# Baverne/VAE-CYCLEGAN-Implementation

Hardware: AMD Instinct MI355X
Metric: train images/sec (256x256 VAE-CycleGAN step) (higher is better)
Workload: dtype f32; 1 GPU; cyclevaegan unpaired, 3x256x256 synthetic summer<->winter, per-GPU batch 8, latent 64 (BASELINE.json configs[3]/[4]); per_gpu_batch=8, global_batch=8, image_size=256, latent_dim=64, parallelism=dp1, init=random (reference init statistics)

## Files before the change

vae-cyclegan-implementation_amd/csrc/conv_igemm.hip:

```cpp
#include "vcg_common.h"
#ifdef VCG_STAMP
#include <stdlib.h>
#endif

struct ConvP {
  const float* a;
  const float* b;
  const float* bias;
  float* out;
  int N, H, W, Cin, Cout, KH, KW, stride, pad, reflect, ups, act;
  int Hl, Wl, Ho, Wo, M, K;
  int cin4, cout4, cout_log;
  FastDiv fd_howo, fd_wo, fd_cin4, fd_cout4, fd_kw, fd_cin;
  int Hc, Wc, Mc, NB;
  FastDiv fd_hcwc, fd_wc;
  int ktiles_total, sk_len, sk_units, sk_ntn, sk_bm_shift, sk_bn_shift;
  int sk_ntr_pb;
  FastDiv fd_sklen;
  int ksplit, kt_per;
  float* slab;
  int adjoint;
  int src_pitch;
  uint32_t a_bytes, b_bytes;
  int dbl_mirror;
// ... 1287 lines not shown
    }
#pragma unroll
    for (int e = 0; e < BE; ++e) {
      vb[e] = bload4(rb, boff[e]);
      if (boff[e] != VCG_OOB) boff[e] += bstep;
    }
  };
  auto store_tiles = [&](int img) {
#pragma unroll
    for (int a = 0; a < AP; ++a) {
      uint2 h, l;
      if (p.a_planes) {
        h = make_uint2(__float_as_uint(va[a].x), __float_as_uint(va[a].y));
        l = make_uint2(__float_as_uint(va[a].z), __float_as_uint(va[a].w));
      } else {
        split4h(va[a], sc.inv_a, h, l);
      }
      const uint32_t o = tr_off<BM>(ps + PS * a, rq * 4);
      *reinterpret_cast<uint2*>(&Xs[img][0][o]) = h;
      *reinterpret_cast<uint2*>(&Xs[img][1][o]) = l;
    }
#pragma unroll
    for (int e = 0; e < BE; ++e) {
      const int idx = tid + NT * e;
      const int pp = idx / (BN / 4), j4 = idx % (BN / 4);
      uint2 h, l;
      split4h(vb[e], sc.inv_b, h, l);
      const uint32_t o = tr_off<BN>(pp, j4 * 4);
      *reinterpret_cast<uint2*>(&Ds[img][0][o]) = h;
      *reinterpret_cast<uint2*>(&Ds[img][1][o]) = l;
    }
  };
  const int tq = (lane & 15) >> 2, tp = lane & 3, tcol = 16 * ((lane >> 4) & 1) + 4 * tp;

  if (kt_begin < kt_end) {
    load_tiles(kt_begin);
    store_tiles(0);
  }
  __syncthreads();
  VCG_STAMP_AT(1);
  for (int kt = kt_begin; kt < kt_end; ++kt) {
    const int img = (kt - kt_begin) & 1;
    if (kt + 1 < kt_end) load_tiles(kt + 1);
#pragma unroll
    for (int s2 = 0; s2 < 2; ++s2) {
      const int row0 = 16 * s2 + 8 * lh + tq;
      f16x8 af[VCG_NP][MI], bfr[VCG_NP][NI];
#pragma unroll
      for (int pc = 0; pc < VCG_NP; ++pc) {
#pragma unroll
        for (int i = 0; i < MI; ++i) af[pc][i] = tr_frag<BM>(Xs[img][pc], row0, wm * (BM / WR) + i * 32 + tcol);
#pragma unroll
        for (int j = 0; j < NI; ++j) bfr[pc][j] = tr_frag<BN>(Ds[img][pc], row0, wn * (BN / 2) + j * 32 + tcol);
      }
#pragma unroll
      for (int i = 0; i < MI; ++i)
#pragma unroll
        for (int j = 0; j < NI; ++j) {
          f32x16 c = lo[i][j];
          c = VCG_MFMA(af[1][i], bfr[0][j], c);
          c = VCG_MFMA(af[0][i], bfr[1][j], c);
          lo[i][j] = c;
          acc[i][j] = VCG_MFMA(af[0][i], bfr[0][j], acc[i][j]);
        }
    }
    if (kt + 1 < kt_end) store_tiles(img ^ 1);
    __syncthreads();
  }
#pragma unroll
  for (int i = 0; i < MI; ++i)
#pragma unroll
    for (int j = 0; j < NI; ++j) acc[i][j] += lo[i][j];
  VCG_STAMP_AT(2);
  const int part = wg - (int)fd_div((uint32_t)(tile * p.ktiles_total), p.fd_sklen);
  float* slab = p.out + ((size_t)part * p.nbatch + zb) * p.K * p.Cout;
#pragma unroll
  for (int j = 0; j < NI; ++j) {
    const int co = n0 + wn * (BN / 2) + j * 32 + l31;
    if (co >= p.Cout) continue;
#pragma unroll
    for (int i = 0; i < MI; ++i) {
#pragma unroll
      for (int e = 0; e < 16; ++e) {
        const int row = (e & 3) + 8 * (e >> 2) + 4 * lh;
        const int Rr = r0 + wm * (BM / WR) + i * 32 + row;
        if (Rr < p.K) slab[(size_t)Rr * p.Cout + co] = acc[i][j][e] * sc.out;
      }
    }
  }
  unit += kt_end - kt_begin;
  if (unit < unit_end) __syncthreads();
  }
  VCG_STAMP_AT(3);
}

__device__ __forceinline__ int sk_parts(const ConvP& p, int R, int co) {
  const int tile = (R >> p.sk_bm_shift) * p.sk_ntn + (co >> p.sk_bn_shift);
  const uint32_t u0 = (uint32_t)(tile * p.ktiles_total);
  return (int)(fd_div(u0 + (uint32_t)p.ktiles_total - 1u, p.fd_sklen) - fd_div(u0, p.fd_sklen)) + 1;
}

__global__ __launch_bounds__(256) void k_slab_sum(const float* __restrict__ slabs, float* __restrict__ out,
                                                  size_t total4, ConvP p, int per_group) {
  const int g = blockIdx.y;
  const int z0 = g * per_group;
  const int c4 = p.Cout / 4;
  for (size_t i = (size_t)blockIdx.x * blockDim.x + threadIdx.x; i < total4; i += (size_t)gridDim.x * blockDim.x) {
    const int R = (int)(i / c4), co = (int)(i - (size_t)R * c4) * 4;
    int z1 = z0 + per_group;
    const int np = sk_parts(p, R, co);
    if (z1 > np) z1 = np;
    float4 s = f4zero();
    for (int z = z0; z < z1; ++z) f4add(s, reinterpret_cast<const float4*>(slabs)[(size_t)z * total4 + i]);
    reinterpret_cast<float4*>(out)[(size_t)g * total4 + i] = s;
  }
}

__global__ __launch_bounds__(256) void k_wgrad_scatter(const float* __restrict__ slabs, float* __restrict__ gw,
                                                       ConvP p, int nsplit, int cin_log, int cout_log) {
  const size_t total = (size_t)p.K * p.Cout;
  const int U2 = p.ups * p.ups, KK = p.KH * p.KW;
  for (size_t idx = (size_t)blockIdx.x * blockDim.x + threadIdx.x; idx < total;
       idx += (size_t)gridDim.x * blockDim.x) {
    const uint32_t R = (uint32_t)(idx / p.Cout);
    const int co = (int)(idx - (size_t)R * p.Cout);
    const uint32_t t = R / (uint32_t)p.Cin;
    const int c = (int)(R - t * (uint32_t)p.Cin);
    if (co >= cout_log || c >= cin_log) continue;
    const int tap9 = (int)t / U2, ph = (int)t - tap9 * U2;
    const int nz = nsplit ? nsplit : sk_parts(p, (int)R, co);
    float s = 0.f;
    for (int z = 0; z < nz; ++z) s += slabs[(size_t)z * total + idx];
    gw[((size_t)co * (cin_log * U2) + (size_t)c * U2 + ph) * KK + tap9] += s;
  }
}

__global__ __launch_bounds__(256) void k_wgrad_scatter_swapped(const float* __restrict__ slabs, float* __restrict__ gw,
                                                               ConvP p, int T, int C, int nsplit, int cin_real,
                                                               int cout_real) {
  const size_t total = (size_t)T * 4 * C;
  for (size_t idx = (size_t)blockIdx.x * blockDim.x + threadIdx.x; idx < total;
       idx += (size_t)gridDim.x * blockDim.x) {
    const int c = (int)(idx % C);
    const int R = (int)(idx / C);
    const int t = R >> 2, j = R & 3;
    if (j >= cout_real || c >= cin_real) continue;
    const int nz = nsplit ? nsplit : sk_parts(p, R, c);
    float s = 0.f;
    for (int z = 0; z < nz; ++z) s += slabs[(size_t)z * total + idx];
    gw[((size_t)j * cin_real + c) * T + t] += s;
  }
}

__global__ __launch_bounds__(256) void k_wgrad_reduce(const float* __restrict__ slabs, float* __restrict__ gw,
                                                      ConvP p, int nsplit, int cin_log, int cout_log) {
  extern __shared__ __attribute__((aligned(16))) float tile[];
  const int U2 = p.ups * p.ups, KK = p.KH * p.KW, T = KK * U2;
  const int co0 = blockIdx.x * 32, c0 = blockIdx.y * 8;
  const int cl_ = threadIdx.x >> 5, col = threadIdx.x & 31;
  const size_t total = (size_t)p.K * p.Cout;
  {
    const int c = c0 + cl_, co = co0 + col;
    const bool ok = c < p.Cin && co < p.Cout;
    for (int t = 0; t < T; ++t) {
      float s = 0.f;
      if (ok) {
        const size_t idx = ((size_t)t * p.Cin + c) * p.Cout + co;
        const int nz = nsplit ? nsplit : sk_parts(p, t * p.Cin + c, co);
        for (int z = 0; z < nz; ++z) s += slabs[(size_t)z * total + idx];
      }
      tile[(t * 8 + cl_) * 33 + col] = s;
    }
  }
  __syncthreads();
  const int wid = threadIdx.x >> 6, lane = threadIdx.x & 63;
  const int cinL = cin_log * U2;
  const int run = 8 * U2 * KK;
  for (int idx = lane; idx < 8 * run; idx += 64) {
    const int j = idx / run, q = idx - j * run;
    const int colw = wid * 8 + j, co = co0 + colw;
    const int clq = q / KK, tap9 = q - clq * KK;
    const int c_local = clq / U2, ph = clq - c_local * U2;
    const int c = c0 + c_local;
    if (co >= cout_log || c >= cin_log) continue;
    const int t = tap9 * U2 + ph;
    const size_t o = ((size_t)co * cinL + (size_t)c * U2 + ph) * KK + tap9;
    gw[o] += tile[(t * 8 + c_local) * 33 + colw];
  }
}

__global__ __launch_bounds__(256) void k_wino_wgrad_reduce(const float* __restrict__ slabs, float* __restrict__ gw, ConvP p,
                                                           int Cin, int ups, int cin_log, int cout_log) {
  __shared__ float tile[9 * 8 * 65];
  const int U2 = ups * ups, KK = 9;
  const int co0 = blockIdx.x * 64, c0 = blockIdx.y * 8, ph = blockIdx.z;
  const int cl_ = threadIdx.x >> 5, col = (threadIdx.x & 31) * 2;
  const size_t plane = (size_t)p.nbatch * p.K * p.Cout;
  {
    const int c = c0 + cl_, co = co0 + col;
    const bool ok = c < Cin;
    float2 s[16];
    int nz[16], nzmax = 0;
#pragma unroll
    for (int xi = 0; xi < 16; ++xi) {
      nz[xi] = ok ? sk_parts(p, xi * p.K + ph * Cin + c, co) : 0;
      nzmax = nz[xi] > nzmax ? nz[xi] : nzmax;
      s[xi] = make_float2(0.f, 0.f);
    }
    const float* src = slabs + (size_t)(ph * Cin + (ok ? c : 0)) * p.Cout + co;
    const size_t xstride = (size_t)p.K * p.Cout;
    for (int z = 0; z < nzmax; ++z) {
      float2 v[16];
#pragma unroll
      for (int xi = 0; xi < 16; ++xi)
        v[xi] = z < nz[xi] ? *reinterpret_cast<const float2*>(src + (size_t)z * plane + (size_t)xi * xstride) : make_float2(0.f, 0.f);
#pragma unroll
      for (int xi = 0; xi < 16; ++xi) { s[xi].x += v[xi].x; s[xi].y += v[xi].y; }
    }
#pragma unroll
    for (int e = 0; e < 2; ++e) {
      float h[3][4];
#pragma unroll
      for (int b = 0; b < 4; ++b) {
        const float s0 = e ? s[0 + b].y : s[0 + b].x, s1 = e ? s[4 + b].y : s[4 + b].x;
        const float s2 = e ? s[8 + b].y : s[8 + b].x, s3 = e ? s[12 + b].y : s[12 + b].x;
        h[0][b] = s0 + 0.5f * (s1 + s2);
        h[1][b] = 0.5f * (s1 - s2);
        h[2][b] = 0.5f * (s1 + s2) + s3;
      }
#pragma unroll
      for (int a = 0; a < 3; ++a) {
        tile[((a * 3 + 0) * 8 + cl_) * 65 + col + e] = h[a][0] + 0.5f * (h[a][1] + h[a][2]);
        tile[((a * 3 + 1) * 8 + cl_) * 65 + col + e] = 0.5f * (h[a][1] - h[a][2]);
        tile[((a * 3 + 2) * 8 + cl_) * 65 + col + e] = 0.5f * (h[a][1] + h[a][2]) + h[a][3];
      }
    }
  }
  __syncthreads();
  const int wid = threadIdx.x >> 6, lane = threadIdx.x & 63;
  const int cinL = cin_log * U2;
  for (int idx = lane; idx < 16 * 8 * KK; idx += 64) {
    const int j = idx / (8 * KK), q = idx - j * (8 * KK);
    const int colw = wid * 16 + j, co = co0 + colw;
    const int c_local = q / KK, tap9 = q - c_local * KK;
    const int c = c0 + c_local;
    if (co >= cout_log || c >= cin_log) continue;
    gw[((size_t)co * cinL + (size_t)c * U2 + ph) * KK + tap9] += tile[(tap9 * 8 + c_local) * 65 + colw];
  }
}

__device__ __forceinline__ void pack_header(const ConvP& p, uint32_t* hdr) {
  if (blockIdx.x == 0 && blockIdx.y == 0 && threadIdx.x < 64) {
    const uint32_t b = vcg_amax_bits(p.amax_b);
    if (threadIdx.x == 0) *hdr = b;
  }
}
__global__ void k_pack_weight(const float* __restrict__ w, float* __restrict__ wf, ConvP p, int cin_log,
                              int cout_log, uint32_t* hdr) {
  pack_header(p, hdr);
  const size_t total = (size_t)p.K * p.Cout;
  for (size_t idx = (size_t)blockIdx.x * blockDim.x + threadIdx.x; idx < total;
       idx += (size_t)gridDim.x * blockDim.x) {
    uint32_t R = (uint32_t)(idx / p.Cout);
    int co = (int)(idx - (size_t)R * p.Cout);
    uint32_t tap = R / (uint32_t)p.Cin;
    int c = (int)(R - tap * (uint32_t)p.Cin);
    float v = 0.f;
    if (co < cout_log && c < cin_log) {
      int ii = 0, jj = 0;
      if (p.ups == 2) { jj = tap & 1; ii = (tap >> 1) & 1; tap >>= 2; }
      int kh = (int)tap / p.KW, kw = (int)tap % p.KW;
      int cl = (p.ups == 2) ? (c * 4 + ii * 2 + jj) : c;
      int cinL = (p.ups == 2) ? cin_log * 4 : cin_log;
      v = w[(((size_t)co * cinL + cl) * p.KH + kh) * p.KW + kw];
    }
    wf[idx] = v;
  }
}

__global__ __launch_bounds__(256) void k_pack_weight_t(const float* __restrict__ w, float* __restrict__ wf, ConvP p,
                                                       int cin_log, int cout_log, uint32_t* hdr) {
  extern __shared__ __attribute__((aligned(16))) float tile[];
  pack_header(p, hdr);
  const int U2 = p.ups * p.ups, KK = p.KH * p.KW, T = KK * U2;
  const int co0 = blockIdx.x * 32, c0 = blockIdx.y * 8;
  const int wid = threadIdx.x >> 6, lane = threadIdx.x & 63;
  const int cinL = cin_log * U2;
  const int run = 8 * U2 * KK;
  for (int j = 0; j < 8; ++j) {
    const int colw = wid * 8 + j, co = co0 + colw;
    for (int q = lane; q < run; q += 64) {
      const int clq = q / KK, tap9 = q - clq * KK;
      const int c_local = clq / U2, ph = clq - c_local * U2;
      const int c = c0 + c_local;
      const int t = tap9 * U2 + ph;
      float v = 0.f;
      if (co < cout_log && c < cin_log) v = w[((size_t)co * cinL + (size_t)c * U2 + ph) * KK + tap9];
      tile[(t * 8 + c_local) * 33 + colw] = v;
    }
  }
  __syncthreads();
  const int cl_ = threadIdx.x >> 5, col = threadIdx.x & 31;
  const int c = c0 + cl_, co = co0 + col;
  if (c < p.Cin && co < p.Cout)
    for (int t = 0; t < T; ++t) wf[((size_t)t * p.Cin + c) * p.Cout + co] = tile[(t * 8 + cl_) * 33 + col];
}

template <bool DGRAD>
__global__ __launch_bounds__(256) void k_pack_planes(const float* __restrict__ w, unsigned short* __restrict__ bp, ConvP p, int cin_log,
                                                     int cout_log) {
  float psc, pinv;
  vcg_scale_of(vcg_amax_bits(p.amax_b), p.amax_b.shift, psc, pinv);
  const int U2 = p.ups * p.ups, KK = p.KH * p.KW;
  const int cinL = cin_log * U2;
  const int KB = (p.K + 31) / 32, CB = p.Cout / 32;
  const size_t total = DGRAD ? (size_t)KK * U2 * p.Cin * (p.Cout / 4) : (size_t)p.Cout * KB * 8;
  for (size_t idx = (size_t)blockIdx.x * blockDim.x + threadIdx.x; idx < total; idx += (size_t)gridDim.x * blockDim.x) {
    float v[4] = {0.f, 0.f, 0.f, 0.f};
    unsigned short* o;
    if (DGRAD) {
      const size_t row = idx / (p.Cout / 4);
      const int co0 = (int)(idx - row * (p.Cout / 4)) * 4;
      const int NB = U2 * p.Cin;
      const int tapfull = (int)(row / NB), J = (int)(row - (size_t)tapfull * NB);
      const int q = J / p.Cin, c = J - q * p.Cin;
      const int kh = tapfull / p.KW, kw = tapfull - kh * p.KW;
      if (c < cin_log) {
#pragma unroll
        for (int e = 0; e < 4; ++e)
          if (co0 + e < cout_log) v[e] = w[(((size_t)(co0 + e) * cinL + (size_t)c * U2 + q) * p.KH + kh) * p.KW + kw];
      }
      o = bp + (row * CB + co0 / 32) * VCG_PBLK + (co0 & 31);
    } else {
      const int co = (int)(idx / ((size_t)KB * 8));
      const int k0 = (int)(idx - (size_t)co * KB * 8) * 4;
      if (co < cout_log && k0 < p.K) {
        uint32_t tap = (uint32_t)k0 / (uint32_t)p.Cin;
        const int c = k0 - (int)tap * p.Cin;
        int ii = 0, jj = 0;
        if (p.ups == 2) { jj = tap & 1; ii = (tap >> 1) & 1; tap >>= 2; }
        const int kh = (int)tap / p.KW, kw = (int)tap % p.KW;
#pragma unroll
        for (int e = 0; e < 4; ++e)
          if (c + e < cin_log) {
            const int cl = (p.ups == 2) ? ((c + e) * 4 + ii * 2 + jj) : c + e;
            v[e] = w[(((size_t)co * cinL + cl) * p.KH + kh) * p.KW + kw];
          }
      }
      o = bp + ((size_t)co * KB + k0 / 32) * VCG_PBLK + (k0 & 31);
    }
    uint2 h, l;
    split4h(make_float4(v[0], v[1], v[2], v[3]), pinv, h, l);
    *reinterpret_cast<uint2*>(o) = h;
    *reinterpret_cast<uint2*>(o + 32) = l;
  }
}

__global__ __launch_bounds__(256) void k_colsum_partial(const float* __restrict__ dy, float* __restrict__ part,
                                                        int M, int C, int rows_per_chunk, int TC) {
  __shared__ float4 red[256];
  const int TP = 256 / TC;
  const int tc = threadIdx.x % TC, tp = threadIdx.x / TC;
  const int c4 = blockIdx.x * TC + tc;
  const int mb = blockIdx.y * rows_per_chunk;
  int me = mb + rows_per_chunk;
  if (me > M) me = M;
  float4 s = make_float4(0.f, 0.f, 0.f, 0.f), s2 = s, s3 = s, s4 = s;
  if (c4 * 4 < C) {
    const float* base = dy + (size_t)c4 * 4;
    int m = mb + tp;
    for (; m + 3 * TP < me; m += 4 * TP) {
      float4 a = ldg4(base + (size_t)m * C), b = ldg4(base + (size_t)(m + TP) * C);
      float4 c = ldg4(base + (size_t)(m + 2 * TP) * C), d = ldg4(base + (size_t)(m + 3 * TP) * C);
      f4add(s, a); f4add(s2, b); f4add(s3, c); f4add(s4, d);
    }
    for (; m < me; m += TP) f4add(s, ldg4(base + (size_t)m * C));
    f4add(s, s2); f4add(s3, s4); f4add(s, s3);
  }
  red[threadIdx.x] = s;
  __syncthreads();
  if (tp == 0 && c4 * 4 < C) {
    for (int k = 1; k < TP; ++k) f4add(s, red[k * TC + tc]);
    float* o = part + (size_t)blockIdx.y * C + c4 * 4;
    *reinterpret_cast<float2*>(o) = make_float2(s.x, s.y);
    *reinterpret_cast<float2*>(o + 2) = make_float2(s.z, s.w);
  }
}
__global__ __launch_bounds__(256) void k_colsum_final(const float* __restrict__ part, float* __restrict__ out, int C,
                                                      int nchunk, int c_log) {
  __shared__ float red[32][8];
  const int il = threadIdx.x & 7, kl = threadIdx.x >> 3;
  const int c = blockIdx.x * 8 + il;
  float s0 = 0.f, s1 = 0.f, s2 = 0.f, s3 = 0.f;
  if (c < c_log) {
    int k = kl;
    for (; k + 96 < nchunk; k += 128) {
      s0 += part[(size_t)k * C + c];
      s1 += part[(size_t)(k + 32) * C + c];
      s2 += part[(size_t)(k + 64) * C + c];
      s3 += part[(size_t)(k + 96) * C + c];
    }
// ... 426 lines not shown
  VCG_CHECK_ARG(pre_mean && pre_rstd, "vcg_conv_fwd_in_pre: null statistics");
  VCG_CHECK_ARG(pre_act >= VCG_ACT_NONE && pre_act <= VCG_ACT_SIGMOID, "vcg_conv_fwd_in_pre: bad activation %d", pre_act);
  const VcgPre pre = {pre_mean, pre_rstd, pre_act};
  (void)vcg_take_hint_x();
  return conv_fwd_in_impl(t_prev, wf, bias, y, mean, rstd, eps, saved, cd, ws, ws_bytes, stream, &pre);
}

extern "C" int vcg_conv_reads_wf(const int32_t* cd) {
  ConvGeom g;
  if (vcg_conv_geom(cd, &g, "vcg_conv_reads_wf")) return 1;
  return (plan_fwd(g).reads_wf || plan_dgrad(g).reads_wf) ? 1 : 0;
}

extern "C" size_t vcg_conv_dgrad_workspace(const int32_t* cd) {
  ConvGeom g;
  if (vcg_conv_geom(cd, &g, "vcg_conv_dgrad_workspace")) return 0;
  return plan_dgrad(g).ws;
}

static KernelRef dgrad_kernel(const DgradPlan& pl) {
  const int bm = pl.t.bm, bn = pl.t.bn;
  if (pl.path == DGRAD_SPLIT_PLANES && bn == 128) return {k_conv_dgrad_split<128, 2>, "k_conv_dgrad_split<128, 2>"};
  if (pl.path == DGRAD_SPLIT_PLANES) return {k_conv_dgrad_split<64, 2>, "k_conv_dgrad_split<64, 2>"};
  if (pl.path == DGRAD_SPLIT32) return {k_conv_dgrad_split<32, 1>, "k_conv_dgrad_split<32, 1>"};
  if (pl.path == DGRAD_SPLIT64_NOPLANES) return {k_conv_dgrad_split<64, 2, false>, "k_conv_dgrad_split<64, 2>"};
  const char* const name = "k_conv_dgrad<fp32 MFMA>";
  if (bn == 32) return {k_conv_dgrad<128, 32, 1>, name};
  if (bm == 128 && bn == 128) return {k_conv_dgrad<128, 128>, name};
  if (bm == 128 && bn == 64) return {k_conv_dgrad<128, 64>, name};
  if (bm == 64 && bn == 128) return {k_conv_dgrad<64, 128>, name};
  return {k_conv_dgrad<64, 64>, name};
}
static void dgrad_setup(const ConvGeom& g, const DgradPlan& pl, void* ws, ConvP& p) {
  p.Hc = g.Hl / g.stride; p.Wc = g.Wl / g.stride; p.Mc = g.N * p.Hc * p.Wc;
  p.NB = g.ups * g.ups * g.Cin;
  p.fd_hcwc = make_fastdiv((uint32_t)(p.Hc * p.Wc));
  p.fd_wc = make_fastdiv((uint32_t)p.Wc);
  auto dbl = [&](int L) { int lo = 1 > L - 1 - g.pad ? 1 : L - 1 - g.pad, hi = g.pad < L - 2 ? g.pad : L - 2; return lo <= hi; };
  p.dbl_mirror = g.reflect && (dbl(g.Hl) || dbl(g.Wl));
  if (pl.t.nsplit > 1) { p.ksplit = pl.t.nsplit; p.kt_per = pl.t.kt_per; p.slab = (float*)ws; }
}

extern "C" int vcg_conv_dgrad(const float* dy, const float* wf, float* dx, const int32_t* cd, void* ws,
                              size_t ws_bytes, void* stream) {
  (void)vcg_take_hint_x();
  const uint64_t dy_handle = vcg_take_hint_dy();
  ConvGeom g;
  if (vcg_conv_geom(cd, &g, "vcg_conv_dgrad")) return -1;
  VCG_CHECK_ARG(dy && wf && dx, "vcg_conv_dgrad: null pointer");
  const DgradPlan pl = plan_dgrad(g);
  VCG_CHECK_ARG(pl.path != DGRAD_UNSUPPORTED, "vcg_conv_dgrad: input %dx%d not divisible by stride", g.Hl, g.Wl);
  VCG_CHECK_ARG(g.stride == 1 || g.ups == 1, "vcg_conv_dgrad: stride 2 with ups 2 unsupported");
  const PackLayout L = pack_layout(g);
  const void* const w_amax = wf + L.hdr;
  hipStream_t st = (hipStream_t)stream;
  if (pl.path == DGRAD_THIN_FOLD) return vcg_thin_fold_dgrad(g, dy, wf + L.wkd, w_amax, dx, ws, ws_bytes, st, dy_handle);
  if (pl.path == DGRAD_THIN) return vcg_thin_dgrad(g, dy, wf, dx, ws, ws_bytes, st);
  if (pl.path == DGRAD_WINO) return vcg_wino_dgrad(g, dy, wf + L.ud, w_amax, dx, ws, ws_bytes, st, dy_handle);
  if (pl.path == DGRAD_SLAB) return vcg_slab_dgrad(g, dy, wf + L.wfd, (L.hdr - L.wfd) * 4, w_amax, dx, ws, ws_bytes, st, dy_handle);
  ConvP p; fill_params(g, p);
  p.a = dy; p.b = wf; p.out = dx;
  if (set_extents(p, (unsigned long long)g.M * g.Cout * 4, (unsigned long long)g.K * g.Cout * 4,
                  "vcg_conv_dgrad: tensor extents must stay below 2 GiB")) return -1;
  const int nsplit = pl.t.nsplit;
  if (nsplit > 1) VCG_CHECK_ARG(ws && ws_bytes >= pl.ws, "vcg_conv_dgrad: workspace too small (%zu)", ws_bytes);
  dgrad_setup(g, pl, ws, p);
  if (pl.path == DGRAD_SPLIT_PLANES) { p.b = wf + L.wfd; p.b_bytes = (uint32_t)((L.hdr - L.wfd) * 4); }
  if (pl.path != DGRAD_FP32) {
    if (vcg_operand_amax(dy, (size_t)g.M * g.Cout, dy_handle, g.reflect ? 4 : 0, st, &p.amax_a)) return -2;
    p.amax_b = vcg_amax_stored(w_amax);
  }
  {
    const KernelRef k = dgrad_kernel(pl);
    dim3 grid((p.Mc + pl.t.bm - 1) / pl.t.bm, (p.NB + pl.t.bn - 1) / pl.t.bn, nsplit * g.stride * g.stride);
    VcgProfScope prof(k.name, 2.0 * g.M * (double)g.K * g.Cout, st);
    hipLaunchKernelGGL(k.fn, grid, dim3(256), 0, st, p);
  }
  if (nsplit > 1)
    hipLaunchKernelGGL(k_splitk_finish, dim3(ew_grid((size_t)g.N * g.H * g.W * g.Cin / 4)), dim3(256), 0, st,
                       (const float*)ws, (const float*)nullptr, dx, (size_t)g.N * g.H * g.W, g.Cin, nsplit, g.Cin,
                       (int)VCG_ACT_NONE);
  VCG_LAUNCH_CHECK("vcg_conv_dgrad");
  return 0;
}

struct WgradPlan { int bm, bn, grid, len, parts, total, ntr, ntn; };
static WgradPlan wgrad_plan(const ConvGeom& g, int batches = 1) {
  WgradPlan best_p = {};
  const int total = (g.M + BK - 1) / BK;
  struct Cand { int bm, bn, resident; double t_step; };
  const Cand cands[4] = {{256, 128, 1, 4.3}, {128, 128, 2, 5.1}, {128, 64, 3, 4.7}, {64, 64, 5, 4.8}};
  double best = 1e30;
  int force = 0;
#ifdef VCG_STAMP
  { const char* e = getenv("VCG_WGRAD_BM"); force = e ? atoi(e) : 0; }
#endif
  for (int ci = 0; ci < 4; ++ci) {
    const Cand& c = cands[ci];
    if (force ? c.bm != force : c.bm == 256) continue;
    if (c.bn == 128 && g.Cout <= 64) continue;
    if (c.bm >= 128 && g.K <= 64) continue;
    if (c.bm == 256 && g.K < 512) continue;
    if (batches > 1 && g.K % c.bm) continue;
    const int ntr = ((g.K + c.bm - 1) / c.bm) * batches, ntn = (g.Cout + c.bn - 1) / c.bn;
    const long long tiles = (long long)ntr * ntn, units = tiles * total;
    if (units >= (1LL << 30)) continue;
    const long long slots = 256LL * c.resident;
    long long len = (units + slots - 1) / slots;
    if (len < 8) len = units < 8 ? units : 8;
    const long long grid = (units + len - 1) / len;
    const int parts = (int)((total + len - 1) / len) + 1;
    double t = (double)len * c.t_step + (double)(grid + tiles) * c.bm * c.bn * 8.0 / 3.0e6;
    if (t < best * 0.97) {
      best = t;
      best_p = {c.bm, c.bn, (int)grid, (int)len, parts, total, ntr, ntn};
    }
  }
  return best_p;
}

static void stream_k_setup(const WgradPlan& wp, ConvP& p) {
  p.ktiles_total = wp.total; p.sk_len = wp.len; p.sk_units = wp.ntr * wp.ntn * wp.total; p.sk_ntn = wp.ntn;
  p.sk_bm_shift = wp.bm == 256 ? 8 : wp.bm == 128 ? 7 : 6; p.sk_bn_shift = wp.bn == 128 ? 7 : 6;
  p.fd_sklen = make_fastdiv((uint32_t)wp.len);
}
static void launch_stream_k(const WgradPlan& wp, const ConvP& p, double flops, hipStream_t st) {
  const int bm = wp.bm, bn = wp.bn;
  const KernelRef k = bm == 128 && bn == 128  ? KernelRef{k_conv_wgrad_split<128>, "k_conv_wgrad_split<128>"}
                      : bm == 128 && bn == 64 ? KernelRef{k_conv_wgrad_split<64>, "k_conv_wgrad_split<64>"}
                      : bm == 64 && bn == 128 ? KernelRef{k_conv_wgrad<64, 128>, "k_conv_wgrad<fp32 MFMA>"}
                      : bm == 64              ? KernelRef{k_conv_wgrad<64, 64>, "k_conv_wgrad<fp32 MFMA>"}
                                              : KernelRef{k_conv_wgrad<256, 128, 512>, "k_conv_wgrad<fp32 MFMA>"};
  VcgProfScope prof(k.name, flops, st);
  hipLaunchKernelGGL(k.fn, dim3(wp.grid), dim3(bm == 256 ? 512 : 256), 0, st, p);
}

static const int kMaxDirectSlabs = 24;

static void colsum_plan(const ConvGeom& g, int& tc, int& cgroups, int& rows, int& nchunk) {
  int c4 = g.Cout / 4;
  tc = 1;
  while (tc * 2 <= c4 && tc * 2 <= 256) tc *= 2;
  cgroups = (c4 + tc - 1) / tc;
  int tp = 256 / tc;
  long long want = 512 / cgroups;
  if (want < 1) want = 1;
  long long r = (g.M + want - 1) / want;
  if (r < 4LL * tp) r = 4LL * tp;
  rows = (int)r;
  nchunk = (g.M + rows - 1) / rows;
}

static ConvGeom wino_gemm_geom(const ConvGeom& g, int T) { return gemm_geom(T, g.ups * g.ups * g.Cin, g.Cout); }
static int wino_wgrad_reduce(const ConvGeom& g, const ConvP& p, const float* dU, float* gw_oihw, hipStream_t st) {
  hipLaunchKernelGGL(k_wino_wgrad_reduce, dim3(g.Cout / 64, (g.Cin + 7) / 8, g.ups * g.ups), dim3(256), 0, st, dU, gw_oihw, p, g.Cin,
                     g.ups, g.cin_log, g.cout_log);
  VCG_LAUNCH_CHECK("vcg_conv_wgrad(winograd reduce)");
  return 0;
}
static size_t wino_core_bytes(const ConvGeom& q, const WgradPlan& wp) { return (size_t)wp.parts * 16 * q.K * q.Cout * sizeof(float) + 256; }
size_t vcg_wino_wgrad_core_workspace(const ConvGeom& g, int T) {
  const ConvGeom q = wino_gemm_geom(g, T);
  return wino_core_bytes(q, wgrad_plan(q, 16));
}
int vcg_wino_wgrad_core(const ConvGeom& g, const float* V, const float* dM, int T, float* gw_oihw, void* ws, size_t ws_bytes,
                        hipStream_t st, const VcgAmax& amax_v, const VcgAmax& amax_dm) {
  const ConvGeom q = wino_gemm_geom(g, T);
  const WgradPlan wp = wgrad_plan(q, 16);
  VCG_CHECK_ARG(wp.grid > 0, "vcg_conv_wgrad: no launch plan for the Winograd path");
  VCG_CHECK_ARG(ws_bytes >= wino_core_bytes(q, wp), "vcg_conv_wgrad: Winograd slab workspace too small");
  ConvP p; fill_params(q, p);
  p.a = V; p.b = dM; p.out = (float*)ws;
  p.amax_a = amax_v; p.amax_b = amax_dm;
  p.a_planes = 1;
  VCG_CHECK_ARG(wp.bm == 128 && q.K % 32 == 0, "vcg_conv_wgrad: pre-split V needs the split-operand tile");
  p.a_bytes = (uint32_t)((size_t)T * q.K * 4); p.b_bytes = (uint32_t)((size_t)T * q.Cout * 4);
  p.nbatch = 16; p.a_bstride = (uint32_t)((size_t)T * q.K); p.b_bstride = (uint32_t)((size_t)T * q.Cout);
  stream_k_setup(wp, p);
  p.sk_ntr_pb = wp.ntr / 16;
  launch_stream_k(wp, p, 2.0 * 16 * (double)T * q.K * q.Cout, st);
  VCG_LAUNCH_CHECK("vcg_conv_wgrad(winograd gemm)");
  return wino_wgrad_reduce(g, p, (const float*)ws, gw_oihw, st);
}

int vcg_wino_wgrad_reduce_one(const ConvGeom& g, const float* dU, float* gw_oihw, hipStream_t st) {
  const ConvGeom q = wino_gemm_geom(g, 32);
  ConvP p; fill_params(q, p);
  p.nbatch = 16;
  p.ktiles_total = 1; p.sk_len = 1; p.sk_ntn = 1; p.sk_bm_shift = 30; p.sk_bn_shift = 30;
  p.fd_sklen = make_fastdiv(1u);
  return wino_wgrad_reduce(g, p, dU, gw_oihw, st);
}

static bool wgrad_swapped_ok(const ConvGeom& g) {
  return g.Cout == 4 && g.stride == 1 && g.ups == 1 && g.Ho == g.H && g.Wo == g.W && g.Cin >= 32;
}
static ConvGeom swapped_geom(const ConvGeom& g) {
  ConvGeom s = g;
  s.Cin = 4; s.Cout = g.Cin; s.cin_log = g.cout_log; s.cout_log = g.cin_log;
  s.taps = g.KH * g.KW; s.K = s.taps * 4; s.M = g.N * g.H * g.W; s.act = 0;
  return s;
}

enum WgradPath { WGRAD_WINO, WGRAD_RING, WGRAD_SWAPPED, WGRAD_STREAM_K };
enum WgradReduce { WRED_SCATTER, WRED_SCATTER_SWAPPED, WRED_REDUCE };
struct WgradWs { size_t slabs_off, slabs_bytes, groups_off, colsum_off, total; };
struct WgradRoute {
  WgradPath path;
  ConvGeom g;
  WgradPlan wp;
  bool slab_sum;
  WgradReduce reduce;
  WgradWs ws;
};
static WgradRoute plan_wgrad(const ConvGeom& g) {
  WgradRoute r = {};
  r.g = g;
  int tc, cgroups, rows, nchunk;
  colsum_plan(g, tc, cgroups, rows, nchunk);
  const size_t cols = (size_t)nchunk * g.Cout * sizeof(float);
  size_t groups = 0;
  if (vcg_wino_wgrad_ok(g)) { r.path = WGRAD_WINO; r.ws.slabs_bytes = vcg_wino_wgrad_workspace(g); }
  else if (vcg_ring_wgrad_ok(g)) { r.path = WGRAD_RING; r.ws.slabs_bytes = vcg_ring_wgrad_workspace(g); }
  else {
    const bool swapped = wgrad_swapped_ok(g);
    r.path = swapped ? WGRAD_SWAPPED : WGRAD_STREAM_K;
    if (swapped) r.g = swapped_geom(g);
    r.wp = wgrad_plan(r.g);
    const size_t totalw = (size_t)r.g.K * r.g.Cout;
    r.ws.slabs_bytes = (size_t)r.wp.parts * totalw * sizeof(float);
    groups = (size_t)16 * totalw * sizeof(float);
    r.slab_sum = r.wp.parts > kMaxDirectSlabs;
    const size_t lds = (size_t)r.g.taps * 8 * 33 * sizeof(float);
    r.reduce = swapped ? WRED_SCATTER_SWAPPED : (totalw < (1u << 20) || lds > 64 * 1024) ? WRED_SCATTER : WRED_REDUCE;
  }
  r.ws.groups_off = up256(r.ws.slabs_bytes);
  r.ws.colsum_off = r.ws.groups_off + up256(groups);
  r.ws.total = r.ws.colsum_off + cols + 1024;
  if (groups) r.ws.total -= r.ws.groups_off - r.ws.slabs_bytes;
  return r;
}

extern "C" size_t vcg_conv_wgrad_workspace(const int32_t* cd) {
  ConvGeom g;
  if (vcg_conv_geom(cd, &g, "vcg_conv_wgrad_workspace")) return 0;
  return plan_wgrad(g).ws.total;
}

static int launch_colsum(const ConvGeom& gorig, const float* dy, float* gbias, float* part, hipStream_t st) {
  int tc, cgroups, rows, nchunk;
  colsum_plan(gorig, tc, cgroups, rows, nchunk);
  hipLaunchKernelGGL(k_colsum_partial, dim3(cgroups, nchunk), dim3(256), 0, st, dy, part, gorig.M, gorig.Cout, rows, tc);
  hipLaunchKernelGGL(k_colsum_final, dim3((gorig.cout_log + 7) / 8), dim3(256), 0, st, (const float*)part, gbias,
                     gorig.Cout, nchunk, gorig.cout_log);
  VCG_LAUNCH_CHECK("vcg_conv_wgrad(bias)");
  return 0;
}

extern "C" int vcg_conv_wgrad_saved(const float* x, const float* dy, float* gw_oihw, float* gbias, const float* saved,
                                    const int32_t* cd, void* ws, size_t ws_bytes, void* stream) {
  const uint64_t x_handle = vcg_take_hint_x(), dy_handle = vcg_take_hint_dy();
  ConvGeom gorig;
  if (vcg_conv_geom(cd, &gorig, "vcg_conv_wgrad")) return -1;
  VCG_CHECK_ARG(x && dy && gw_oihw && ws, "vcg_conv_wgrad: null pointer");
  const WgradRoute r = plan_wgrad(gorig);
  VCG_CHECK_ARG(ws_bytes >= r.ws.total, "vcg_conv_wgrad: workspace %zu < %zu", ws_bytes, r.ws.total);
  hipStream_t st = (hipStream_t)stream;
  float* const colsum = (float*)((char*)ws + r.ws.colsum_off);
  if (r.path == WGRAD_WINO || r.path == WGRAD_RING) {
    if (r.path == WGRAD_WINO ? vcg_wino_wgrad(gorig, x, dy, gw_oihw, ws, r.ws.slabs_bytes, st, saved, x_handle, dy_handle)
                             : vcg_ring_wgrad(gorig, x, dy, gw_oihw, ws, r.ws.slabs_bytes, st, x_handle, dy_handle))
      return -2;
    return gbias ? launch_colsum(gorig, dy, gbias, colsum, st) : 0;
  }
  const bool swapped = r.path == WGRAD_SWAPPED;
  const ConvGeom& g = r.g;
  const WgradPlan& wp = r.wp;
  ConvP p; fill_params(g, p);
  p.a = x; p.b = dy; p.out = (float*)((char*)ws + r.ws.slabs_off);
  if (swapped) { p.a = dy; p.b = x; p.adjoint = 1; p.src_pitch = 4; }
  if (set_extents(p, swapped ? (unsigned long long)gorig.M * 4 * 4 : (unsigned long long)g.N * g.H * g.W * g.Cin * 4,
                  (unsigned long long)g.M * g.Cout * 4, "vcg_conv_wgrad: tensor extents must stay below 2 GiB")) return -1;
  stream_k_setup(wp, p);
  if (wp.bm == 128) {
    if (vcg_operand_amax(p.a, (size_t)p.a_bytes / 4, swapped ? dy_handle : x_handle, (swapped && gorig.reflect) ? 4 : 0, st, &p.amax_a) ||
        vcg_operand_amax(p.b, (size_t)p.b_bytes / 4, swapped ? x_handle : dy_handle, 0, st, &p.amax_b))
      return -2;
  }
  launch_stream_k(wp, p, 2.0 * g.M * (double)g.K * g.Cout, st);
  VCG_LAUNCH_CHECK("vcg_conv_wgrad");
  const size_t totalw = (size_t)g.K * g.Cout;
  const float* src = p.out;
  int ns = 0;
  if (r.slab_sum) {
    float* grp = (float*)((char*)ws + r.ws.groups_off);
    int per_group = (wp.parts + 15) / 16;
    int G = (wp.parts + per_group - 1) / per_group;
    size_t total4 = totalw / 4;
    int bx = (int)((total4 + 255) / 256); if (bx > 1024) bx = 1024;
    hipLaunchKernelGGL(k_slab_sum, dim3(bx, G), dim3(256), 0, st, src, grp, total4, p, per_group);
    src = grp;
    ns = G;
  }
  int blocks = (int)((totalw + 255) / 256); if (blocks > 4096) blocks = 4096;
  if (r.reduce == WRED_SCATTER_SWAPPED)
    hipLaunchKernelGGL(k_wgrad_scatter_swapped, dim3(blocks), dim3(256), 0, st, src, gw_oihw, p, g.KH * g.KW, g.Cout, ns,
                       gorig.cin_log, gorig.cout_log);
  else if (r.reduce == WRED_SCATTER)
    hipLaunchKernelGGL(k_wgrad_scatter, dim3(blocks), dim3(256), 0, st, src, gw_oihw, p, ns, g.cin_log, g.cout_log);
  else
    hipLaunchKernelGGL(k_wgrad_reduce, dim3((g.Cout + 31) / 32, (g.Cin + 7) / 8), dim3(256), (size_t)g.taps * 8 * 33 * sizeof(float),
                       st, src, gw_oihw, p, ns, g.cin_log, g.cout_log);
  VCG_LAUNCH_CHECK("vcg_conv_wgrad(reduce)");
  return gbias ? launch_colsum(gorig, dy, gbias, colsum, st) : 0;
}
extern "C" int vcg_conv_wgrad(const float* x, const float* dy, float* gw_oihw, float* gbias,
                              const int32_t* cd, void* ws, size_t ws_bytes, void* stream) {
  return vcg_conv_wgrad_saved(x, dy, gw_oihw, gbias, nullptr, cd, ws, ws_bytes, stream);
}
```

Baseline: 256.1 images/s.

## Restage wgrad reduce tiles in output order for vectorized aligned gradient accumulation

Rewrites the weight-gradient reduce kernels so the shared-memory tile is laid out in the destination OIHW order, with per-row alignment phase padding. A shared helper can then accumulate into the gradient with float4 read-modify-writes instead of scattered scalar adds. The generic reduce also batches 8 taps per slab pass. The Winograd reduce now covers all phases in one block with float4 loads and gains a specialized single-part variant that skips the split bookkeeping. This targets uncoalesced global writes and the extra launch dimension, at the cost of more complex index math and a risk of alignment or edge-case bugs.

New measurement: 253.8 images/s. Within noise of the previous version (-0.9%).

```diff
diff --git a/vae-cyclegan-implementation_amd/csrc/conv_igemm.hip b/vae-cyclegan-implementation_amd/csrc/conv_igemm.hip
--- a/vae-cyclegan-implementation_amd/csrc/conv_igemm.hip
+++ b/vae-cyclegan-implementation_amd/csrc/conv_igemm.hip
@@ -1463,101 +1463,150 @@
   }
 }
 
+__device__ __forceinline__ int wgrad_tile_row(int j, int pitch) { return j * pitch + 4 * (j >> 3); }
+__device__ __forceinline__ float f4at(const float4& v, int e) { return e == 0 ? v.x : e == 1 ? v.y : e == 2 ? v.z : v.w; }
+__device__ __forceinline__ int wgrad_run_phase(const float* gw, size_t base) {
+  return (int)(((reinterpret_cast<uintptr_t>(gw) >> 2) + base) & 3);
+}
+__device__ __forceinline__ void wgrad_tile_accumulate(float* __restrict__ gw, const float* tile, int nco, int pitch, int co0,
+                                                      int cout_log, size_t co_stride, size_t blk_off, int elim) {
+  const int Q = pitch >> 2;
+  int j = threadIdx.x / Q, m = threadIdx.x - j * Q;
+  while (j < nco) {
+    const int co = co0 + j;
+    if (co < cout_log) {
+      const size_t base = (size_t)co * co_stride + blk_off;
+      const int a = wgrad_run_phase(gw, base);
+      const int lo = a, hi = a + elim, q = 4 * m;
+      const float* t = tile + wgrad_tile_row(j, pitch) + q;
+      float* g = gw + base - a + q;
+      if (q >= lo && q + 4 <= hi) {
+        float4 o = *reinterpret_cast<float4*>(g);
+        const float4 v = *reinterpret_cast<const float4*>(t);
+        o.x += v.x; o.y += v.y; o.z += v.z; o.w += v.w;
+        *reinterpret_cast<float4*>(g) = o;
+      } else {
+#pragma unroll
+        for (int i = 0; i < 4; ++i)
+          if (q + i >= lo && q + i < hi) g[i] += t[i];
+      }
+    }
+    m += 256;
+    while (m >= Q) { m -= Q; ++j; }
+  }
+}
+
+static size_t wgrad_reduce_lds(int T) { return (size_t)(32 * (8 * T + 4) + 16) * sizeof(float); }
 __global__ __launch_bounds__(256) void k_wgrad_reduce(const float* __restrict__ slabs, float* __restrict__ gw,
                                                       ConvP p, int nsplit, int cin_log, int cout_log) {
   extern __shared__ __attribute__((aligned(16))) float tile[];
   const int U2 = p.ups * p.ups, KK = p.KH * p.KW, T = KK * U2;
+  const int ush = p.ups == 2 ? 2 : 0;
   const int co0 = blockIdx.x * 32, c0 = blockIdx.y * 8;
   const int cl_ = threadIdx.x >> 5, col = threadIdx.x & 31;
   const size_t total = (size_t)p.K * p.Cout;
+  const int pitch = 8 * T + 4;
+  const size_t co_stride = (size_t)cin_log * T, blk_off = (size_t)c0 * T;
   {
     const int c = c0 + cl_, co = co0 + col;
     const bool ok = c < p.Cin && co < p.Cout;
-    for (int t = 0; t < T; ++t) {
-      float s = 0.f;
-      if (ok) {
-        const size_t idx = ((size_t)t * p.Cin + c) * p.Cout + co;
-        const int nz = nsplit ? nsplit : sk_parts(p, t * p.Cin + c, co);
-        for (int z = 0; z < nz; ++z) s += slabs[(size_t)z * total + idx];
-      }
-      tile[(t * 8 + cl_) * 33 + col] = s;
+    float* dst = tile + wgrad_tile_row(col, pitch) + wgrad_run_phase(gw, (size_t)co * co_stride + blk_off) + cl_ * T;
+    for (int t0 = 0; t0 < T; t0 += 8) {
+      float s[8];
+      int nz[8], nzmax = 0;
+#pragma unroll
+      for (int u = 0; u < 8; ++u) {
+        const int t = t0 + u;
+        nz[u] = (ok && t < T) ? (nsplit ? nsplit : sk_parts(p, t * p.Cin + c, co)) : 0;
+        nzmax = nz[u] > nzmax ? nz[u] : nzmax;
+        s[u] = 0.f;
+      }
+      const float* src = slabs + ((size_t)t0 * p.Cin + (ok ? c : 0)) * p.Cout + (ok ? co : 0);
+      const size_t tstride = (size_t)p.Cin * p.Cout;
+      for (int z = 0; z < nzmax; ++z) {
+        float v[8];
+#pragma unroll
+        for (int u = 0; u < 8; ++u) v[u] = z < nz[u] ? src[(size_t)z * total + (size_t)u * tstride] : 0.f;
+#pragma unroll
+        for (int u = 0; u < 8; ++u) s[u] += v[u];
+      }
+#pragma unroll
+      for (int u = 0; u < 8; ++u) {
+        const int t = t0 + u;
+        if (t < T) dst[(t & (U2 - 1)) * KK + (t >> ush)] = s[u];
+      }
     }
   }
   __syncthreads();
-  const int wid = threadIdx.x >> 6, lane = threadIdx.x & 63;
-  const int cinL = cin_log * U2;
-  const int run = 8 * U2 * KK;
-  for (int idx = lane; idx < 8 * run; idx += 64) {
-    const int j = idx / run, q = idx - j * run;
-    const int colw = wid * 8 + j, co = co0 + colw;
-    const int clq = q / KK, tap9 = q - clq * KK;
-    const int c_local = clq / U2, ph = clq - c_local * U2;
-    const int c = c0 + c_local;
-    if (co >= cout_log || c >= cin_log) continue;
-    const int t = tap9 * U2 + ph;
-    const size_t o = ((size_t)co * cinL + (size_t)c * U2 + ph) * KK + tap9;
-    gw[o] += tile[(t * 8 + c_local) * 33 + colw];
-  }
-}
-
+  int elim = (cin_log - c0) * T;
+  elim = elim < 0 ? 0 : elim > 8 * T ? 8 * T : elim;
+  wgrad_tile_accumulate(gw, tile, 32, pitch, co0, cout_log, co_stride, blk_off, elim);
+}
+
+constexpr int kWinoRedPitch = 32 * 9 + 4;
+template <bool ONE>
 __global__ __launch_bounds__(256) void k_wino_wgrad_reduce(const float* __restrict__ slabs, float* __restrict__ gw, ConvP p,
                                                            int Cin, int ups, int cin_log, int cout_log) {
-  __shared__ float tile[9 * 8 * 65];
+  __shared__ __attribute__((aligned(16))) float tile[32 * kWinoRedPitch + 12];
   const int U2 = ups * ups, KK = 9;
-  const int co0 = blockIdx.x * 64, c0 = blockIdx.y * 8, ph = blockIdx.z;
-  const int cl_ = threadIdx.x >> 5, col = (threadIdx.x & 31) * 2;
+  const int co0 = blockIdx.x * 32, c0 = blockIdx.y * (32 / U2);
+  const int r = threadIdx.x >> 3, col = (threadIdx.x & 7) * 4;
+  const int cl_ = ups == 2 ? r >> 2 : r, ph = ups == 2 ? r & 3 : 0;
   const size_t plane = (size_t)p.nbatch * p.K * p.Cout;
+  const size_t co_stride = (size_t)cin_log * U2 * KK, blk_off = (size_t)c0 * U2 * KK;
   {
     const int c = c0 + cl_, co = co0 + col;
     const bool ok = c < Cin;
-    float2 s[16];
-    int nz[16], nzmax = 0;
-#pragma unroll
-    for (int xi = 0; xi < 16; ++xi) {
-      nz[xi] = ok ? sk_parts(p, xi * p.K + ph * Cin + c, co) : 0;
-      nzmax = nz[xi] > nzmax ? nz[xi] : nzmax;
-      s[xi] = make_float2(0.f, 0.f);
-    }
+    float4 s[16];
     const float* src = slabs + (size_t)(ph * Cin + (ok ? c : 0)) * p.Cout + co;
     const size_t xstride = (size_t)p.K * p.Cout;
-    for (int z = 0; z < nzmax; ++z) {
-      float2 v[16];
-#pragma unroll
-      for (int xi = 0; xi < 16; ++xi)
-        v[xi] = z < nz[xi] ? *reinterpret_cast<const float2*>(src + (size_t)z * plane + (size_t)xi * xstride) : make_float2(0.f, 0.f);
-#pragma unroll
-      for (int xi = 0; xi < 16; ++xi) { s[xi].x += v[xi].x; s[xi].y += v[xi].y; }
-    }
-#pragma unroll
-    for (int e = 0; e < 2; ++e) {
+    if (ONE) {
+#pragma unroll
+      for (int xi = 0; xi < 16; ++xi) {
+        const float4 v = ok ? *reinterpret_cast<const float4*>(src + (size_t)xi * xstride) : f4zero();
+        s[xi].x = 0.f + v.x; s[xi].y = 0.f + v.y; s[xi].z = 0.f + v.z; s[xi].w = 0.f + v.w;
+      }
+    } else {
+      int nz[16], nzmax = 0;
+#pragma unroll
+      for (int xi = 0; xi < 16; ++xi) {
+        nz[xi] = ok ? sk_parts(p, xi * p.K + ph * Cin + c, co) : 0;
+        nzmax = nz[xi] > nzmax ? nz[xi] : nzmax;
+        s[xi] = f4zero();
+      }
+      for (int z = 0; z < nzmax; ++z) {
+        float4 v[16];
+#pragma unroll
+        for (int xi = 0; xi < 16; ++xi)
+          v[xi] = z < nz[xi] ? *reinterpret_cast<const float4*>(src + (size_t)z * plane + (size_t)xi * xstride) : f4zero();
+#pragma unroll
+        for (int xi = 0; xi < 16; ++xi) { s[xi].x += v[xi].x; s[xi].y += v[xi].y; s[xi].z += v[xi].z; s[xi].w += v[xi].w; }
+      }
+    }
+#pragma unroll
+    for (int e = 0; e < 4; ++e) {
       float h[3][4];
 #pragma unroll
       for (int b = 0; b < 4; ++b) {
-        const float s0 = e ? s[0 + b].y : s[0 + b].x, s1 = e ? s[4 + b].y : s[4 + b].x;
-        const float s2 = e ? s[8 + b].y : s[8 + b].x, s3 = e ? s[12 + b].y : s[12 + b].x;
+        const float s0 = f4at(s[0 + b], e), s1 = f4at(s[4 + b], e);
+        const float s2 = f4at(s[8 + b], e), s3 = f4at(s[12 + b], e);
         h[0][b] = s0 + 0.5f * (s1 + s2);
         h[1][b] = 0.5f * (s1 - s2);
         h[2][b] = 0.5f * (s1 + s2) + s3;
       }
+      float* dst = tile + wgrad_tile_row(col + e, kWinoRedPitch) + wgrad_run_phase(gw, (size_t)(co + e) * co_stride + blk_off) + r * KK;
 #pragma unroll
       for (int a = 0; a < 3; ++a) {
-        tile[((a * 3 + 0) * 8 + cl_) * 65 + col + e] = h[a][0] + 0.5f * (h[a][1] + h[a][2]);
-        tile[((a * 3 + 1) * 8 + cl_) * 65 + col + e] = 0.5f * (h[a][1] - h[a][2]);
-        tile[((a * 3 + 2) * 8 + cl_) * 65 + col + e] = 0.5f * (h[a][1] + h[a][2]) + h[a][3];
+        dst[a * 3 + 0] = h[a][0] + 0.5f * (h[a][1] + h[a][2]);
+        dst[a * 3 + 1] = 0.5f * (h[a][1] - h[a][2]);
+        dst[a * 3 + 2] = 0.5f * (h[a][1] + h[a][2]) + h[a][3];
       }
     }
   }
   __syncthreads();
-  const int wid = threadIdx.x >> 6, lane = threadIdx.x & 63;
-  const int cinL = cin_log * U2;
-  for (int idx = lane; idx < 16 * 8 * KK; idx += 64) {
-    const int j = idx / (8 * KK), q = idx - j * (8 * KK);
-    const int colw = wid * 16 + j, co = co0 + colw;
-    const int c_local = q / KK, tap9 = q - c_local * KK;
-    const int c = c0 + c_local;
-    if (co >= cout_log || c >= cin_log) continue;
-    gw[((size_t)co * cinL + (size_t)c * U2 + ph) * KK + tap9] += tile[(tap9 * 8 + c_local) * 65 + colw];
-  }
+  int elim = (cin_log - c0) * U2 * KK;
+  elim = elim < 0 ? 0 : elim > 32 * KK ? 32 * KK : elim;
+  wgrad_tile_accumulate(gw, tile, 32, kWinoRedPitch, co0, cout_log, co_stride, blk_off, elim);
 }
 
 __device__ __forceinline__ void pack_header(const ConvP& p, uint32_t* hdr) {
@@ -2290,9 +2339,13 @@
 }
 
 static ConvGeom wino_gemm_geom(const ConvGeom& g, int T) { return gemm_geom(T, g.ups * g.ups * g.Cin, g.Cout); }
-static int wino_wgrad_reduce(const ConvGeom& g, const ConvP& p, const float* dU, float* gw_oihw, hipStream_t st) {
-  hipLaunchKernelGGL(k_wino_wgrad_reduce, dim3(g.Cout / 64, (g.Cin + 7) / 8, g.ups * g.ups), dim3(256), 0, st, dU, gw_oihw, p, g.Cin,
-                     g.ups, g.cin_log, g.cout_log);
+static int wino_wgrad_reduce(const ConvGeom& g, const ConvP& p, const float* dU, float* gw_oihw, bool one_part, hipStream_t st) {
+  const int cb = 32 / (g.ups * g.ups);
+  const dim3 grid(g.Cout / 32, (g.Cin + cb - 1) / cb);
+  if (one_part)
+    hipLaunchKernelGGL(k_wino_wgrad_reduce<true>, grid, dim3(256), 0, st, dU, gw_oihw, p, g.Cin, g.ups, g.cin_log, g.cout_log);
+  else
+    hipLaunchKernelGGL(k_wino_wgrad_reduce<false>, grid, dim3(256), 0, st, dU, gw_oihw, p, g.Cin, g.ups, g.cin_log, g.cout_log);
   VCG_LAUNCH_CHECK("vcg_conv_wgrad(winograd reduce)");
   return 0;
 }
@@ -2318,7 +2371,7 @@
   p.sk_ntr_pb = wp.ntr / 16;
   launch_stream_k(wp, p, 2.0 * 16 * (double)T * q.K * q.Cout, st);
   VCG_LAUNCH_CHECK("vcg_conv_wgrad(winograd gemm)");
-  return wino_wgrad_reduce(g, p, (const float*)ws, gw_oihw, st);
+  return wino_wgrad_reduce(g, p, (const float*)ws, gw_oihw, false, st);
 }
 
 int vcg_wino_wgrad_reduce_one(const ConvGeom& g, const float* dU, float* gw_oihw, hipStream_t st) {
@@ -2327,7 +2380,7 @@
   p.nbatch = 16;
   p.ktiles_total = 1; p.sk_len = 1; p.sk_ntn = 1; p.sk_bm_shift = 30; p.sk_bn_shift = 30;
   p.fd_sklen = make_fastdiv(1u);
-  return wino_wgrad_reduce(g, p, dU, gw_oihw, st);
+  return wino_wgrad_reduce(g, p, dU, gw_oihw, true, st);
 }
 
 static bool wgrad_swapped_ok(const ConvGeom& g) {
@@ -2447,8 +2500,8 @@
   else if (r.reduce == WRED_SCATTER)
     hipLaunchKernelGGL(k_wgrad_scatter, dim3(blocks), dim3(256), 0, st, src, gw_oihw, p, ns, g.cin_log, g.cout_log);
   else
-    hipLaunchKernelGGL(k_wgrad_reduce, dim3((g.Cout + 31) / 32, (g.Cin + 7) / 8), dim3(256), (size_t)g.taps * 8 * 33 * sizeof(float),
-                       st, src, gw_oihw, p, ns, g.cin_log, g.cout_log);
+    hipLaunchKernelGGL(k_wgrad_reduce, dim3((g.Cout + 31) / 32, (g.Cin + 7) / 8), dim3(256), wgrad_reduce_lds(g.taps), st, src, gw_oihw,
+                       p, ns, g.cin_log, g.cout_log);
   VCG_LAUNCH_CHECK("vcg_conv_wgrad(reduce)");
   return gbias ? launch_colsum(gorig, dy, gbias, colsum, st) : 0;
 }
```
